# Ghostish/Open3DSOT

Hardware: NVIDIA H100
Metric: template-search pairs/sec, BAT-Car fwd+bwd (higher is better)
Workload: dtype f32

## Files before the change

### open3dsot_b200/csrc/pwmlp_tc.cu

```cuda
#include <type_traits>
#include "common.cuh"
#include "lift.cuh"
#include "tc_ptx.cuh"
#include "../../include/o3d_b200.h"

namespace {

struct TcAct {
    const float* x; int ld; const float* scale; const float* shift; int relu;
    struct Coef { float4 s, t; bool on; };
    template <int R> struct Batch { float4 v[R]; };
    __device__ __forceinline__ Coef prep(int k, int K) const {
        Coef c;
        c.on = k < K;
        c.s = make_float4(1.f, 1.f, 1.f, 1.f);
        c.t = make_float4(0.f, 0.f, 0.f, 0.f);
        if (c.on && scale) { c.s = ld4g(scale + k); c.t = ld4g(shift + k); }
        return c;
    }
    template <int R>
    __device__ __forceinline__ void fetch(Batch<R>& b, int p0, int stride, int P, int k, int K) const {
        const int kk = k < K ? k : 0;
#pragma unroll
        for (int i = 0; i < R; ++i) {
// ... 210 lines not shown
                s2 = fmaf(v[j], v[j], s2);
            }
            if (S > 0) {
                float gm = v[0], gn = v[0];
                int ga = 0, gb = 0;
#pragma unroll
                for (int j = 1; j < 16; ++j) {
                    if (v[j] > gm) { gm = v[j]; ga = j; }
                    if (v[j] < gn) { gn = v[j]; gb = j; }
                }
                const int s0 = pbase & smask;
                if (s0 == 0) { mx = gm; ax = ga; mn = gn; an = gb; }
                else {
                    if (gm > mx) { mx = gm; ax = s0 + ga; }
                    if (gn < mn) { mn = gn; an = s0 + gb; }
                }
                if (s0 + 16 == S) {
                    const size_t o = (size_t)(pbase >> log2S) * ldp + ch;
                    ymax[o] = mx; ymin[o] = mn; arg[o] = ax | (an << 16);
                }
            }
        } else {
#pragma unroll
            for (int j = 0; j < 16; ++j) {
                if (pbase + j >= P) break;
                const float v = __uint_as_float(r[j]) + bv;
                if (yp) yp[(size_t)j * ldy] = v;
                s1 += v;
                s2 = fmaf(v, v, s2);
                if (S > 0) {
                    const int s = (pbase + j) & smask;
                    if (s == 0) { mx = -INFINITY; mn = INFINITY; ax = an = 0; }
                    if (v > mx) { mx = v; ax = s; }
                    if (v < mn) { mn = v; an = s; }
                    if (s == smask) {
                        const size_t o = (size_t)((pbase + j) >> log2S) * ldp + ch;
                        ymax[o] = mx; ymin[o] = mn; arg[o] = ax | (an << 16);
                    }
                }
            }
        }
        d1 += (double)s1;
        d2 += (double)s2;
    }
    __device__ __forceinline__ void end(int ch, int Nw) {
        if (sum && ch < Nw) {
            atomicAdd(sum + ch, d1);
            atomicAdd(sumsq + ch, d2);
        }
    }
};

template <int LD, bool LIFT = false>
struct TcDgradEpi {
    float* out; int ldo; const float* yprev; int ldyp; const float* scale; const float* shift; int relu;
    double* s1g; double* s2y;
    LiftView lv;
    float sc, sh; double d1, d2;
    float yv[16];
    float u0, u1, u2, u3; const int32_t* gs; const float4* ss;
    __device__ __forceinline__ bool lifted() const { return LIFT; }
    __device__ __forceinline__ void begin(int ch, int Nw) {
        d1 = d2 = 0.0;
        sc = (scale && ch < Nw) ? scale[ch] : 1.f;
        sh = (shift && ch < Nw) ? shift[ch] : 0.f;
        if constexpr (LIFT) {
            const bool on = lv.u && ch < Nw;
            u0 = on ? lv.u[ch] : 0.f; u1 = on ? lv.u[lv.ldz + ch] : 0.f; u2 = on ? lv.u[2 * lv.ldz + ch] : 0.f; u3 = on ? lv.u[3 * lv.ldz + ch] : 0.f;
            gs = nullptr;
        }
    }
    __device__ __forceinline__ const int32_t* lift_gidx() const { return LIFT ? lv.gidx : nullptr; }
    __device__ __forceinline__ const float* lift_s() const { return LIFT ? lv.s : nullptr; }
    __device__ __forceinline__ void set_tile(const int32_t* g, const float4* s4) { if constexpr (LIFT) { gs = g; ss = s4; } }
    __device__ __forceinline__ void prefetch_lift(int ch, int pbase, int col, int P) {
#pragma unroll
        for (int j = 0; j < 16; ++j) {
            const float z = lv.z ? __ldg(lv.z + (size_t)gs[col + j] * lv.ldz + ch) : 0.f;
            const float4 sv = lv.s ? ss[col + j] : make_float4(0.f, 0.f, 0.f, 0.f);
            yv[j] = lift_val(z, sv, u0, u1, u2, u3);
        }
    }
    __device__ __forceinline__ void prefetch(int ch, int Nw, int pbase, int P) {
        if (ch >= Nw) return;
        if constexpr (LIFT) { prefetch_lift(ch, pbase, pbase & (TC_N - 1), P); return; }
        if (!yprev) return;
        if (pbase + 16 <= P) {
            const float* yp = yprev + (size_t)pbase * ldyp + ch;
            const size_t st = LD ? (size_t)LD : (size_t)ldyp;
#pragma unroll
            for (int j = 0; j < 16; ++j) yv[j] = __ldg(yp + j * st);
        } else {
#pragma unroll
            for (int j = 0; j < 16; ++j) {
                const int pj = min(pbase + j, P - 1);
                yv[j] = __ldg(yprev + (size_t)pj * ldyp + ch);
            }
        }
    }
    __device__ __forceinline__ void group(const uint32_t (&r)[16], int ch, int Nw, int pbase, int P) {
        if (ch >= Nw) return;
        float s1 = 0.f, s2 = 0.f;
        float* op = out + (size_t)pbase * ldo + ch;
        if (pbase + 16 <= P) {
            float v[16];
#pragma unroll
            for (int j = 0; j < 16; ++j) v[j] = __uint_as_float(r[j]);
            if (yprev || lifted()) {
                if (relu) {
#pragma unroll
                    for (int j = 0; j < 16; ++j) v[j] = fmaf(yv[j], sc, sh) > 0.f ? v[j] : 0.f;
                }
#pragma unroll
                for (int j = 0; j < 16; ++j) s2 = fmaf(v[j], yv[j], s2);
            }
            const size_t st = LD ? (size_t)LD : (size_t)ldo;
#pragma unroll
            for (int j = 0; j < 16; ++j) {
                s1 += v[j];
                op[j * st] = v[j];
            }
        } else {
#pragma unroll
            for (int j = 0; j < 16; ++j) {
                if (pbase + j >= P) break;
                float v = __uint_as_float(r[j]);
                if (yprev || lifted()) {
                    if (relu && !(fmaf(yv[j], sc, sh) > 0.f)) v = 0.f;
                    s2 = fmaf(v, yv[j], s2);
                }
                s1 += v;
                op[(size_t)j * ldo] = v;
            }
        }
        d1 += (double)s1;
        d2 += (double)s2;
    }
    __device__ __forceinline__ void end(int ch, int Nw) {
        if (s1g && ch < Nw) {
            atomicAdd(s1g + ch, d1);
            atomicAdd(s2y + ch, d2);
        }
    }
};

constexpr int TC_STAGES = 2;
constexpr int TC_STAGE_BYTES = 4 * TILE_BYTES;
constexpr int TC_EPI_LD = 68;
constexpr int TC_EPI_BYTES = TC_M * TC_EPI_LD * 4;
constexpr int TC_THREADS = 512;
constexpr int TC_SMEM = TC_STAGES * TC_STAGE_BYTES + 2 * TC_EPI_BYTES + 1024 + 256 + 1024 + 4096;

template <int R>
__device__ __forceinline__ void stage_acc(const float (&acc)[R], float* stg, int ld) {
    const int w = (threadIdx.x >> 5) & 3, lane = threadIdx.x & 31;
#pragma unroll
    for (int i = 0; i < R; ++i) {
        const int row = 16 * w + (lane >> 2) + 8 * ((i >> 1) & 1), col = 8 * (i >> 2) + 2 * (lane & 3) + (i & 1);
        stg[col * ld + row] = acc[i];
    }
}

template <class BLoad, class Epi>
__global__ void __launch_bounds__(TC_THREADS, 1)
    pw_tc_kernel(BLoad bl, const uint8_t* __restrict__ wtiles, int P, int K, int Nw, int nkb, Epi epi, int rev) {
    constexpr bool BF = is_bf16<BLoad>::value;
    constexpr int WBYTES = BF ? BF_TILE_BYTES : 2 * TILE_BYTES;
    extern __shared__ uint8_t smem_raw[];
    uint8_t* smem = reinterpret_cast<uint8_t*>((reinterpret_cast<uintptr_t>(smem_raw) + 1023) & ~(uintptr_t)1023);
    uint8_t* tail = smem + TC_STAGES * TC_STAGE_BYTES + 2 * TC_EPI_BYTES;
    uint64_t* full = reinterpret_cast<uint64_t*>(tail);
    uint64_t* empty = full + TC_STAGES;

    const int warp = threadIdx.x >> 5, lane = threadIdx.x & 31;
    const int mt0 = blockIdx.y;
    const int n_ptiles = (P + TC_N - 1) / TC_N;
    auto tile_of = [&](int t) { return rev ? n_ptiles - 1 - t : t; };

    if (threadIdx.x == 0) {
        for (int s = 0; s < TC_STAGES; ++s) {
            o3d_mbar_init(full + s, 256 + 1);
            o3d_mbar_init(empty + s, 8);
        }
        o3d_fence_mbar_init();
    }
    __syncthreads();

    if (warp < 8) {
        const int h = warp >> 2;
        const int tw = threadIdx.x & 127;
        const int ch = mt0 * TC_M + tw;
        float* stg = reinterpret_cast<float*>(smem + TC_STAGES * TC_STAGE_BYTES + h * TC_EPI_BYTES);
        int32_t* gsm = reinterpret_cast<int32_t*>(tail + 256);
        float4* ssm = reinterpret_cast<float4*>(tail + 256 + 1024);
        epi.begin(ch, Nw);
        int stage = 0, phase = 0, buf = 0;
        for (int t = blockIdx.x; t < n_ptiles; t += gridDim.x) {
            const int pt0 = tile_of(t) * TC_N;
            {
                const int32_t* gi = epi.lift_gidx();
                const float* si = epi.lift_s();
                if (gi || si) {
                    const int pp = min(pt0 + tw, P - 1);
                    if (gi && h == 0) gsm[buf * TC_N + tw] = __ldg(gi + pp);
                    if (si && h == 1) ssm[buf * TC_N + tw] = ld4g(si + (size_t)pp * 4);
                    asm volatile("bar.sync 1, 256;" ::: "memory");
                    epi.set_tile(gsm + buf * TC_N, ssm + buf * TC_N);
                }
            }
            const int pb = pt0 + h * 64;
            epi.prefetch(ch, Nw, pb, P);
            float acc[64];
#pragma unroll
            for (int i = 0; i < 64; ++i) acc[i] = 0.f;
            for (int kb = 0; kb < nkb; ++kb) {
                o3d_mbar_wait(full + stage, phase);
                const uint32_t sb = o3d_smem_u32(smem + stage * TC_STAGE_BYTES);
                wgmma_fence_acc(acc);
                wgmma_fence();
                if constexpr (BF) {
                    const uint32_t xb = sb + 2 * TILE_BYTES + h * (BF_TILE_BYTES / 2);
                    wgmma_bf16_kblock<128>(acc, make_desc_sw64(xb), make_desc_sw64(sb), kb == 0);
                } else {
                    const uint32_t xb = sb + 2 * TILE_BYTES + h * (TILE_BYTES / 2);
                    wgmma_3xtf32_kblock<128>(acc, make_desc(xb), make_desc(xb + TILE_BYTES), make_desc(sb), make_desc(sb + TILE_BYTES),
                                             kb == 0);
                }
                wgmma_commit();
                wgmma_wait<0>();
                wgmma_fence_acc(acc);
                if (lane == 0) o3d_mbar_arrive(empty + stage);
                if (++stage == TC_STAGES) { stage = 0; phase ^= 1; }
            }
            asm volatile("bar.sync %0, 128;" ::"r"(2 + h) : "memory");
            stage_acc(acc, stg, TC_EPI_LD);
            asm volatile("bar.sync %0, 128;" ::"r"(2 + h) : "memory");
            const float* row = stg + tw * TC_EPI_LD;
#pragma unroll 1
            for (int cg = 0; cg < 4; ++cg) {
                uint32_t r[16];
#pragma unroll
                for (int j = 0; j < 4; ++j) {
                    const float4 v = *reinterpret_cast<const float4*>(row + cg * 16 + 4 * j);
                    r[4 * j] = __float_as_uint(v.x); r[4 * j + 1] = __float_as_uint(v.y);
                    r[4 * j + 2] = __float_as_uint(v.z); r[4 * j + 3] = __float_as_uint(v.w);
                }
                epi.group(r, ch, Nw, pb + cg * 16, P);
                if (cg + 1 < 4) epi.prefetch(ch, Nw, pb + (cg + 1) * 16, P);
            }
            buf ^= 1;
        }
        epi.end(ch, Nw);
    } else {
        const int pt = (warp - 8) * 32 + lane;
        const int chunk = pt & 7;
        const int row0 = (pt >> 3) * 4;
        int stage = 0, phase = 0;
        struct Cur { int t, kb, p0; };
        auto advance = [&](Cur& c) {
            if (++c.kb == nkb) {
                c.kb = 0;
                c.t += gridDim.x;
                if (c.t < n_ptiles) c.p0 = tile_of(c.t) * TC_N;
            }
        };
        using Batch4 = typename BLoad::template Batch<4>;
        auto issue = [&](Batch4& r, typename BLoad::Coef& cf, const Cur& c) {
            if (c.t >= n_ptiles) return;
            const int k = c.kb * TC_K + chunk * 4;
            cf = bl.prep(k, K);
            bl.fetch(r, c.p0 + row0, 1, P, k, K);
        };
        Cur c0{(int)blockIdx.x, 0, 0};
        if (c0.t < n_ptiles) c0.p0 = tile_of(c0.t) * TC_N;
        Batch4 r0{};
        typename BLoad::Coef f0 = bl.prep(chunk * 4, K);
        issue(r0, f0, c0);
        if (pt == 0 && c0.t < n_ptiles) bl.prefetch_rows(c0.p0, TC_N, P);
        while (c0.t < n_ptiles) {
            o3d_mbar_wait(empty + stage, phase ^ 1);
            if (pt == 0) {
                o3d_mbar_expect_tx(full + stage, WBYTES);
                o3d_bulk_g2s(smem + stage * TC_STAGE_BYTES, wtiles + ((size_t)mt0 * nkb + c0.kb) * WBYTES, WBYTES, full + stage);
                const int tn = c0.t + (int)gridDim.x;
                if (c0.kb == 0 && tn < n_ptiles) bl.prefetch_rows(tile_of(tn) * TC_N, TC_N, P);
            }
            uint8_t* xhi = smem + stage * TC_STAGE_BYTES + 2 * TILE_BYTES;
            uint8_t* xlo = xhi + TILE_BYTES;
#pragma unroll
            for (int i = 0; i < 4; ++i) {
                const float4 v = bl.finish(r0, f0, i, c0.p0 + row0 + i, P);
                if constexpr (BF) {
                    *reinterpret_cast<uint2*>(xhi + sw64(row0 + i, chunk >> 1) + (chunk & 1) * 8) = pack_bf16x4(v);
                } else {
                    const uint32_t off = sw128(row0 + i, chunk);
                    *reinterpret_cast<float4*>(xhi + off) = hi_part(v);
                    *reinterpret_cast<float4*>(xlo + off) = lo_part(v);
                }
            }
            o3d_fence_proxy_async();
            o3d_mbar_arrive(full + stage);
            if (++stage == TC_STAGES) { stage = 0; phase ^= 1; }
            advance(c0);
            issue(r0, f0, c0);
        }
    }
}

constexpr int WG_STAGES = 3;
constexpr int WG_AHEAD = 4;
constexpr int WG_THREADS = 512;
constexpr int WG_SMEM = WG_STAGES * 4 * TILE_BYTES + 1024 + 256;

template <class L>
__device__ __forceinline__ void store_transposed(const L& ld, const typename L::template Batch<4>& raw, const typename L::Coef& cf,
                                                 uint8_t* hi, int c_local, int p_first, int prow0, int pend) {
#pragma unroll
    for (int i = 0; i < 4; ++i) {
        const int pl = prow0 + 8 * i;
        const float4 v = ld.finish(raw, cf, i, p_first + pl, pend);
        const float e[4] = {v.x, v.y, v.z, v.w};
#pragma unroll
        for (int j = 0; j < 4; ++j) {
            const uint32_t off = sw128(c_local + j, pl >> 2) + (uint32_t)((pl & 3) * 4);
            const float h = hi1(e[j]);
            *reinterpret_cast<float*>(hi + off) = h;
            *reinterpret_cast<float*>(hi + TILE_BYTES + off) = e[j] - h;
        }
    }
}

constexpr int WG_BF_SUB = TC_K * TC_BF_ROW;
constexpr int WG_BF_X = 4 * WG_BF_SUB;

template <class L>
__device__ __forceinline__ void store_rows_bf16(const L& ld, const typename L::template Batch<4>& raw, const typename L::Coef& cf,
                                                uint8_t* img, int sub, int c_local, int p_first, int prow0, int pend) {
#pragma unroll
    for (int i = 0; i < 4; ++i) {
        const int pl = prow0 + 8 * i;
        st_bf16_row4(img, sub, pl, c_local, ld.finish(raw, cf, i, p_first + pl, pend));
    }
}

template <class XB>
__global__ void __launch_bounds__(WG_THREADS, 1)
    pw_wgrad_tc_kernel(TcDy da, XB xb, int P, int M, int N, int chunk, float* __restrict__ part) {
    constexpr bool BF = is_bf16<XB>::value;
    extern __shared__ uint8_t smem_raw[];
    uint8_t* smem = reinterpret_cast<uint8_t*>((reinterpret_cast<uintptr_t>(smem_raw) + 1023) & ~(uintptr_t)1023);
    uint64_t* full = reinterpret_cast<uint64_t*>(smem + WG_STAGES * 4 * TILE_BYTES);
    uint64_t* empty = full + WG_STAGES;

    const int warp = threadIdx.x >> 5, lane = threadIdx.x & 31;
    const int m0 = blockIdx.z * TC_M, n0 = blockIdx.y * TC_N;
    const int pbeg = blockIdx.x * chunk, pend = min(P, pbeg + chunk);
    const int nkb = pend > pbeg ? (pend - pbeg + TC_K - 1) / TC_K : 0;
    auto kpos = [&](int i) { return pbeg + i * TC_K; };

    if (threadIdx.x == 0) {
        for (int s = 0; s < WG_STAGES; ++s) {
            o3d_mbar_init(full + s, 256);
            o3d_mbar_init(empty + s, 8);
        }
        o3d_fence_mbar_init();
    }
    __syncthreads();

    if (warp < 8) {
        const int h = warp >> 2, w = warp & 3;
        float acc[64];
#pragma unroll
        for (int i = 0; i < 64; ++i) acc[i] = 0.f;
        int stage = 0, phase = 0;
        for (int kb = 0; kb < nkb; ++kb) {
            o3d_mbar_wait(full + stage, phase);
            const uint32_t sb = o3d_smem_u32(smem + stage * 4 * TILE_BYTES);
            wgmma_fence_acc(acc);
            wgmma_fence();
            if constexpr (BF) {
                const uint32_t ab = sb + h * 2 * WG_BF_SUB;
#pragma unroll
                for (int ks = 0; ks < 2; ++ks)
                    wgmma_bf16_tt_n128(acc, make_desc_sw64_mn(ab + ks * 1024, WG_BF_SUB),
                                       make_desc_sw64_mn(sb + WG_BF_X + ks * 1024, WG_BF_SUB), (kb == 0 && ks == 0) ? 0u : 1u);
            } else {
                const uint32_t ab = sb + h * (TILE_BYTES / 2);
                wgmma_3xtf32_kblock<128>(acc, make_desc(ab), make_desc(ab + TILE_BYTES), make_desc(sb + 2 * TILE_BYTES),
                                         make_desc(sb + 3 * TILE_BYTES), kb == 0);
            }
            wgmma_commit();
            wgmma_wait<0>();
            wgmma_fence_acc(acc);
            if (lane == 0) o3d_mbar_arrive(empty + stage);
            if (++stage == WG_STAGES) { stage = 0; phase ^= 1; }
        }
        const int Mt = TC_M * (int)gridDim.z, Nt = TC_N * (int)gridDim.y;
        float* __restrict__ out = part + (size_t)blockIdx.x * Mt * Nt;
#pragma unroll
        for (int i = 0; i < 64; i += 4) {
#pragma unroll
            for (int rr = 0; rr < 2; ++rr) {
                const int m = m0 + h * 64 + 16 * w + (lane >> 2) + 8 * rr, n = n0 + 8 * (i >> 2) + 2 * (lane & 3);
                *reinterpret_cast<float2*>(out + (size_t)m * Nt + n) = make_float2(acc[i + 2 * rr], acc[i + 2 * rr + 1]);
            }
        }
    } else {
        const int pw = warp - 8;
        const int c4 = pw * 4 + (lane & 3), prow0 = lane >> 2;
        const bool pt0 = pw == 0 && lane == 0;
        TcDy::Batch<4> ra = {};
        typename XB::template Batch<4> rb = {};
        auto fetch = [&](int kb) {
            da.fetch(ra, kpos(kb) + prow0, 8, pend, m0 + c4 * 4, M);
            xb.fetch(rb, kpos(kb) + prow0, 8, pend, n0 + c4 * 4, N);
        };
        auto prefetch = [&](int kb) {
            if (pt0 && kb < nkb) {
                da.prefetch_rows(kpos(kb), TC_K, pend);
                xb.prefetch_rows(kpos(kb), TC_K, pend);
            }
        };
        int stage = 0, phase = 0;
        for (int kb = 0; kb < WG_AHEAD; ++kb) prefetch(kb);
        if (nkb > 0) fetch(0);
        for (int kb = 0; kb < nkb; ++kb) {
            prefetch(kb + WG_AHEAD);
            o3d_mbar_wait(empty + stage, phase ^ 1);
            uint8_t* sbase = smem + stage * 4 * TILE_BYTES;
            if constexpr (BF) {
                store_rows_bf16(da, ra, da.prep(m0 + c4 * 4, M), sbase, WG_BF_SUB, c4 * 4, kpos(kb), prow0, pend);
                store_rows_bf16(xb, rb, xb.prep(n0 + c4 * 4, N), sbase + WG_BF_X, WG_BF_SUB, c4 * 4, kpos(kb), prow0, pend);
            } else {
                store_transposed(da, ra, da.prep(m0 + c4 * 4, M), sbase, c4 * 4, kpos(kb), prow0, pend);
                store_transposed(xb, rb, xb.prep(n0 + c4 * 4, N), sbase + 2 * TILE_BYTES, c4 * 4, kpos(kb), prow0, pend);
            }
            o3d_fence_proxy_async();
            o3d_mbar_arrive(full + stage);
            if (kb + 1 < nkb) fetch(kb + 1);
            if (++stage == WG_STAGES) { stage = 0; phase ^= 1; }
        }
    }
}

__global__ void __launch_bounds__(256)
    wgrad_reduce_kernel(const float* __restrict__ part, int splits, int Mt, int Nt, int M, int N, float* __restrict__ dW,
                        int lddw) {
    const int sub = threadIdx.x & 7;
    const int n4 = (blockIdx.x * 32 + (threadIdx.x >> 3)) * 4, m = blockIdx.y;
    float4 acc = make_float4(0.f, 0.f, 0.f, 0.f);
    if (n4 < N && m < M) {
        const float* p = part + (size_t)m * Nt + n4;
        for (int s = sub; s < splits; s += 8) {
            const float4 v = __ldg(reinterpret_cast<const float4*>(p + (size_t)s * Mt * Nt));
            acc.x += v.x; acc.y += v.y; acc.z += v.z; acc.w += v.w;
        }
    }
#pragma unroll
    for (int o = 4; o >= 1; o >>= 1) {
        acc.x += __shfl_xor_sync(0xFFFFFFFFu, acc.x, o); acc.y += __shfl_xor_sync(0xFFFFFFFFu, acc.y, o);
        acc.z += __shfl_xor_sync(0xFFFFFFFFu, acc.z, o); acc.w += __shfl_xor_sync(0xFFFFFFFFu, acc.w, o);
    }
    if (sub == 0 && n4 < N && m < M) {
        float* o = dW + (size_t)m * lddw + n4;
        o[0] += acc.x;
        if (n4 + 1 < N) o[1] += acc.y;
        if (n4 + 2 < N) o[2] += acc.z;
        if (n4 + 3 < N) o[3] += acc.w;
    }
}

constexpr int BW_TP = 64;
constexpr int BW_THREADS = 384;
constexpr int BW_DY = 0, BW_XT = 64 * 1024, BW_W = 128 * 1024, BW_TAIL = 192 * 1024;
constexpr int BW_SMEM = BW_TAIL + 256 + 1024 + 4096 + 1024;
constexpr int BW_BF_SUB = BW_TP * TC_BF_ROW;

template <class XB, int N>
__global__ void __launch_bounds__(BW_THREADS, 1)
    pw_bwd_tc_kernel(TcDy da, XB xb, const uint8_t* __restrict__ wtiles, int P, int M, TcDgradEpi<N, is_lift<XB>::value> epi,
                     float* __restrict__ part) {
    constexpr bool BF = is_bf16<XB>::value;
    constexpr int NH = N / 2;
    constexpr int WSTAGE = BF ? NH * TC_BF_ROW : 2 * NH * 128;
    extern __shared__ uint8_t smem_raw[];
    uint8_t* smem = reinterpret_cast<uint8_t*>((reinterpret_cast<uintptr_t>(smem_raw) + 1023) & ~(uintptr_t)1023);
    uint8_t* tail = smem + BW_TAIL;
    uint64_t* dy_full = reinterpret_cast<uint64_t*>(tail);
    uint64_t* dy_empty = dy_full + 1;
    uint64_t* xt_full = dy_full + 2;
    uint64_t* xt_empty = dy_full + 3;
    uint64_t* wfull = dy_full + 4;

    const int warp = threadIdx.x >> 5, lane = threadIdx.x & 31;
    const int nkb = M / TC_K;
    const int n_ptiles = (P + BW_TP - 1) / BW_TP;
    const int my_tiles = blockIdx.x < n_ptiles ? (n_ptiles - 1 - blockIdx.x) / gridDim.x + 1 : 0;

    if (threadIdx.x == 0) {
        o3d_mbar_init(dy_full, 128);
        o3d_mbar_init(dy_empty, 8);
        o3d_mbar_init(xt_full, 128);
        o3d_mbar_init(xt_empty, 8);
        for (int s = 0; s < 4; ++s) o3d_mbar_init(wfull + s, 1);
        o3d_fence_mbar_init();
    }
    __syncthreads();

    if (warp < 8) {
        const int h = warp >> 2, w = warp & 3, tw = threadIdx.x & 127;
        uint8_t* wring = smem + BW_W + h * 2 * WSTAGE;
        const int n_witems = my_tiles * nkb;
        auto load_w = [&](int item) {
            const int s = item & 1;
            o3d_mbar_expect_tx(wfull + 2 * h + s, WSTAGE);
            if constexpr (BF) {
                const uint8_t* src = wtiles + (size_t)(item % nkb) * BF_TILE_BYTES + h * NH * TC_BF_ROW;
                o3d_bulk_g2s(wring + s * WSTAGE, src, WSTAGE, wfull + 2 * h + s);
            } else {
                const uint8_t* src = wtiles + (size_t)(item % nkb) * (2 * TILE_BYTES) + h * NH * 128;
                o3d_bulk_g2s(wring + s * WSTAGE, src, NH * 128, wfull + 2 * h + s);
                o3d_bulk_g2s(wring + s * WSTAGE + NH * 128, src + TILE_BYTES, NH * 128, wfull + 2 * h + s);
            }
        };
        if (tw == 0) {
            if (n_witems > 0) load_w(0);
            if (n_witems > 1) load_w(1);
        }
        const bool do_w = 64 * h < M;
        const int n_local = h * NH + (tw % NH);
        const int q = tw / NH;
        constexpr int PPT = NH / 2;
        float* stg = reinterpret_cast<float*>(smem + BW_XT + h * (NH * TC_EPI_LD * 4));
        int32_t* gsm = reinterpret_cast<int32_t*>(tail + 256);
        float4* ssm = reinterpret_cast<float4*>(tail + 256 + 1024);
        epi.begin(n_local, N);
        float wacc[N / 2];
#pragma unroll
        for (int i = 0; i < N / 2; ++i) wacc[i] = 0.f;
        int witem = 0, tphase = 0, buf = 0;
        for (int t = blockIdx.x; t < n_ptiles; t += gridDim.x) {
            const int pt0 = t * BW_TP;
            {
                const int32_t* gi = epi.lift_gidx();
                const float* si = epi.lift_s();
                if (gi || si) {
                    if (tw < BW_TP) {
                        const int pp = min(pt0 + tw, P - 1);
                        const int slot = buf * TC_N + ((pt0 + tw) & (TC_N - 1));
                        if (gi && h == 0) gsm[slot] = __ldg(gi + pp);
                        if (si && h == 1) ssm[slot] = ld4g(si + (size_t)pp * 4);
                    }
                    asm volatile("bar.sync 1, 256;" ::: "memory");
                    epi.set_tile(gsm + buf * TC_N, ssm + buf * TC_N);
                }
            }
            const int pb = pt0 + q * PPT;
            float dacc[NH / 2];
#pragma unroll
            for (int i = 0; i < NH / 2; ++i) dacc[i] = 0.f;
            o3d_mbar_wait(dy_full, tphase);
            for (int kb = 0; kb < nkb; ++kb, ++witem) {
                o3d_mbar_wait(wfull + 2 * h + (witem & 1), (witem >> 1) & 1);
                const uint32_t bb = o3d_smem_u32(wring + (witem & 1) * WSTAGE);
                wgmma_fence_acc(dacc);
                wgmma_fence();
                if constexpr (BF) {
                    wgmma_bf16_kblock<NH>(dacc, make_desc_sw64(o3d_smem_u32(smem + BW_DY + kb * BW_BF_SUB)), make_desc_sw64(bb), kb == 0);
                } else {
                    const uint32_t ab = o3d_smem_u32(smem + BW_DY + kb * TILE_BYTES);
                    wgmma_3xtf32_kblock<NH>(dacc, make_desc(ab), make_desc(ab + TILE_BYTES / 2), make_desc(bb), make_desc(bb + NH * 128),
                                            kb == 0);
                }
                wgmma_commit();
                wgmma_wait<0>();
                wgmma_fence_acc(dacc);
                asm volatile("bar.sync %0, 128;" ::"r"(2 + h) : "memory");
                if (tw == 0 && witem + 2 < n_witems) load_w(witem + 2);
            }
            o3d_mbar_wait(xt_full, tphase);
            if constexpr (BF) {
                if (do_w) {
                    const uint32_t ab = o3d_smem_u32(smem + BW_DY + 2 * h * BW_BF_SUB), xb0 = o3d_smem_u32(smem + BW_XT);
                    wgmma_fence_acc(wacc);
                    wgmma_fence();
#pragma unroll
                    for (int ks = 0; ks < BW_TP / 16; ++ks) {
                        const uint64_t ad = make_desc_sw64_mn(ab + ks * 1024, BW_BF_SUB), bd = make_desc_sw64_mn(xb0 + ks * 1024, BW_BF_SUB);
                        if constexpr (N == 128) wgmma_bf16_tt_n128(wacc, ad, bd, 1u);
                        else wgmma_bf16_tt_n64(wacc, ad, bd, 1u);
                    }
                    wgmma_commit();
                    wgmma_wait<0>();
                    wgmma_fence_acc(wacc);
                }
            } else if (do_w) {
                const int mr = 16 * w + (lane >> 2);
                const uint8_t* dyk = smem + BW_DY + (2 * h + (w >> 1)) * (TILE_BYTES);
                const int mc = mr & 31;
                const uint32_t xt = o3d_smem_u32(smem + BW_XT);
#pragma unroll 1
                for (int ks = 0; ks < BW_TP / 8; ++ks) {
                    uint32_t ahi[4], alo[4];
#pragma unroll
                    for (int i = 0; i < 4; ++i) {
                        const int p = ks * 8 + (lane & 3) + 4 * (i >> 1), m = mc + 8 * (i & 1);
                        const uint32_t off = sw128(p, m >> 2) + 4 * (m & 3);
                        ahi[i] = *reinterpret_cast<const uint32_t*>(dyk + off);
                        alo[i] = *reinterpret_cast<const uint32_t*>(dyk + TILE_BYTES / 2 + off);
                    }
                    const uint32_t xb0 = xt + (ks >> 2) * (2 * TILE_BYTES) + (ks & 3) * 32;
                    const uint64_t bhi = make_desc(xb0), blo = make_desc(xb0 + TILE_BYTES);
                    wgmma_fence_acc(wacc);
                    wgmma_fence();
                    if constexpr (N == 128) {
                        wgmma_tf32_rs_n128(wacc, alo, bhi);
                        wgmma_tf32_rs_n128(wacc, ahi, blo);
                        wgmma_tf32_rs_n128(wacc, ahi, bhi);
                    } else {
                        wgmma_tf32_rs_n64(wacc, alo, bhi);
                        wgmma_tf32_rs_n64(wacc, ahi, blo);
                        wgmma_tf32_rs_n64(wacc, ahi, bhi);
                    }
                    wgmma_commit();
                    wgmma_wait<0>();
                    wgmma_fence_acc(wacc);
                }
            }
            __syncwarp();
            if (lane == 0) o3d_mbar_arrive(dy_empty);
            epi.prefetch(n_local, N, pb, P);
            asm volatile("bar.sync 4, 256;" ::: "memory");
            stage_acc(dacc, stg, TC_EPI_LD);
            asm volatile("bar.sync %0, 128;" ::"r"(2 + h) : "memory");
            const float* row = stg + (tw % NH) * TC_EPI_LD + q * PPT;
#pragma unroll 1
            for (int cg = 0; cg < PPT / 16; ++cg) {
                uint32_t r[16];
#pragma unroll
                for (int j = 0; j < 4; ++j) {
                    const float4 v = *reinterpret_cast<const float4*>(row + cg * 16 + 4 * j);
                    r[4 * j] = __float_as_uint(v.x); r[4 * j + 1] = __float_as_uint(v.y);
                    r[4 * j + 2] = __float_as_uint(v.z); r[4 * j + 3] = __float_as_uint(v.w);
                }
                epi.group(r, n_local, N, pb + cg * 16, P);
                if (cg + 1 < PPT / 16) epi.prefetch(n_local, N, pb + (cg + 1) * 16, P);
            }
            __syncwarp();
            if (lane == 0) o3d_mbar_arrive(xt_empty);
            tphase ^= 1;
            buf ^= 1;
        }
        epi.end(n_local, N);
        if (do_w) {
            float* __restrict__ out = part + (size_t)blockIdx.x * TC_M * TC_N;
#pragma unroll
            for (int i = 0; i < N / 2; i += 4) {
#pragma unroll
                for (int rr = 0; rr < 2; ++rr) {
                    const int m = 64 * h + 16 * w + (lane >> 2) + 8 * rr, n = 8 * (i >> 2) + 2 * (lane & 3);
                    *reinterpret_cast<float2*>(out + (size_t)m * TC_N + n) = make_float2(wacc[i + 2 * rr], wacc[i + 2 * rr + 1]);
                }
            }
        }
    } else {
        const int pt = threadIdx.x - 256;
        const int chunk = pt & 7, row0 = (pt >> 3) * 4;
        const int pw = warp - 8, c4 = pw * 4 + (lane & 3), prow0 = lane >> 2;
        constexpr int NXH = N / 64;
        const int n_items_x = 2 * NXH;
        struct It { int t, i; };
        TcDy::Batch<4> ra{};
        typename XB::template Batch<4> rb{};
        It ca{(int)blockIdx.x, 0}, cb{(int)blockIdx.x, 0};
        auto fetch_a = [&](const It& c) {
            if (c.t < n_ptiles) da.fetch(ra, c.t * BW_TP + row0, 1, P, c.i * TC_K + chunk * 4, M);
        };
        auto fetch_b = [&](const It& c) {
            if (c.t < n_ptiles)
                xb.fetch(rb, c.t * BW_TP + (c.i >> (NXH - 1)) * TC_K + prow0, 8, P, (c.i & (NXH - 1)) * 64 + c4 * 4, N);
        };
        fetch_a(ca);
        fetch_b(cb);
        if (pt == 0 && ca.t < n_ptiles) { da.prefetch_rows(ca.t * BW_TP, BW_TP, P); xb.prefetch_rows(ca.t * BW_TP, BW_TP, P); }
        int tphase = 0;
        for (int t = blockIdx.x; t < n_ptiles; t += gridDim.x) {
            const int pt0 = t * BW_TP;
            if (pt == 0) {
                const int tn = t + (int)gridDim.x;
                if (tn < n_ptiles) { da.prefetch_rows(tn * BW_TP, BW_TP, P); xb.prefetch_rows(tn * BW_TP, BW_TP, P); }
            }
            o3d_mbar_wait(dy_empty, tphase ^ 1);
            for (int kb = 0; kb < nkb; ++kb) {
                const int k = kb * TC_K + chunk * 4;
                const TcDy::Coef cf = da.prep(k, M);
                if constexpr (BF) {
#pragma unroll
                    for (int i = 0; i < 4; ++i)
                        st_bf16_row4(smem + BW_DY + kb * BW_BF_SUB, 0, row0 + i, chunk * 4, da.finish(ra, cf, i, pt0 + row0 + i, P));
                } else {
                    uint8_t* hi = smem + BW_DY + kb * TILE_BYTES;
#pragma unroll
                    for (int i = 0; i < 4; ++i) {
                        const float4 v = da.finish(ra, cf, i, pt0 + row0 + i, P);
                        const uint32_t off = sw128(row0 + i, chunk);
                        *reinterpret_cast<float4*>(hi + off) = hi_part(v);
                        *reinterpret_cast<float4*>(hi + TILE_BYTES / 2 + off) = lo_part(v);
                    }
                }
                if (++ca.i == nkb) { ca.i = 0; ca.t += gridDim.x; }
                fetch_a(ca);
            }
            o3d_fence_proxy_async();
            o3d_mbar_arrive(dy_full);
            o3d_mbar_wait(xt_empty, tphase ^ 1);
            for (int it = 0; it < n_items_x; ++it) {
                const int j = it >> (NXH - 1), cl = (it & (NXH - 1)) * 64 + c4 * 4;
                if constexpr (BF)
                    store_rows_bf16(xb, rb, xb.prep(cl, N), smem + BW_XT + j * (TC_K * TC_BF_ROW), BW_BF_SUB, cl, pt0 + j * TC_K, prow0, P);
                else
                    store_transposed(xb, rb, xb.prep(cl, N), smem + BW_XT + j * (2 * TILE_BYTES), cl, pt0 + j * TC_K, prow0, P);
                if (++cb.i == n_items_x) { cb.i = 0; cb.t += gridDim.x; }
                fetch_b(cb);
            }
            o3d_fence_proxy_async();
            o3d_mbar_arrive(xt_full);
            tphase ^= 1;
        }
    }
}

__global__ void w_pretile_kernel(const float* __restrict__ W, int ld, int rows, int K, int nkb, uint8_t* __restrict__ out) {
    const int m_tile = blockIdx.y, kb = blockIdx.x;
    uint8_t* dst = out + ((size_t)m_tile * nkb + kb) * (2 * TILE_BYTES);
    for (int id = threadIdx.x; id < TC_M * 8; id += blockDim.x) {
        const int r = id >> 3, c = id & 7;
        const int row = m_tile * TC_M + r, k = kb * TC_K + c * 4;
        float4 v = make_float4(0.f, 0.f, 0.f, 0.f);
        if (row < rows && k < K) v = *reinterpret_cast<const float4*>(W + (size_t)row * ld + k);
        const uint32_t off = sw128(r, c);
        *reinterpret_cast<float4*>(dst + off) = hi_part(v);
        *reinterpret_cast<float4*>(dst + TILE_BYTES + off) = lo_part(v);
    }
}

inline int ilog2_exact(int v) { int l = 0; while ((1 << l) < v) ++l; return l; }

template <class BLoad, class Epi>
int launch_tc(BLoad bl, const uint8_t* wtiles, int P, int K, int Nw, Epi epi, bool reverse, cudaStream_t st, const char* name) {
    auto kern = pw_tc_kernel<BLoad, Epi>;
    O3D_CUDA(cudaFuncSetAttribute(kern, cudaFuncAttributeMaxDynamicSharedMemorySize, TC_SMEM), name);
    const int gy = (Nw + TC_M - 1) / TC_M;
    const int nkb = (K + TC_K - 1) / TC_K;
    const int n_ptiles = (P + TC_N - 1) / TC_N;
    int gx = o3d_num_sms() / gy;
    if (gx < 1) gx = 1;
    if (gx > n_ptiles) gx = n_ptiles;
    kern<<<dim3(gx, gy), TC_THREADS, TC_SMEM, st>>>(bl, wtiles, P, K, Nw, nkb, epi, reverse);
    O3D_CHECK_LAUNCH(name);
    return O3D_OK;
}

template <int LD, class BLoad>
int launch_fwd(const BLoad& bl, const void* wtiles, const float* bias, int P, int K, int Nw, float* y, int ldy, double* sum,
               double* sumsq, int S, float* ymax, float* ymin, int32_t* arg, int ldp, bool reverse, cudaStream_t st) {
    TcFwdEpi<LD> ep{};
    ep.y = y; ep.ldy = ldy; ep.bias = bias; ep.sum = sum; ep.sumsq = sumsq;
    ep.S = S; ep.ymax = ymax; ep.ymin = ymin; ep.arg = arg; ep.ldp = ldp;
    ep.log2S = 0;
    while ((1 << ep.log2S) < S) ++ep.log2S;
    return launch_tc(bl, (const uint8_t*)wtiles, P, K, Nw, ep, reverse, st, "o3d_pw_fwd_tc");
}

template <int LD, bool LIFT = false, class BL>
int launch_dgrad(const BL& bl, const void* wtiles_t, int P, int Cout, int Cin, float* out, int ldo, const float* yprev,
                 int ldyp, const float* pscale, const float* pshift, int prelu, double* s1, double* s2y, cudaStream_t st,
                 const LiftView* lv = nullptr) {
    if constexpr (!LIFT) {
        if (lv) return launch_dgrad<LD, true>(bl, wtiles_t, P, Cout, Cin, out, ldo, yprev, ldyp, pscale, pshift, prelu, s1, s2y, st, lv);
    }
    TcDgradEpi<LD, LIFT> ep{};
    if (lv) ep.lv = *lv;
    ep.out = out; ep.ldo = ldo; ep.yprev = yprev; ep.ldyp = ldyp; ep.scale = pscale; ep.shift = pshift; ep.relu = prelu;
    ep.s1g = s1; ep.s2y = s2y;
    return launch_tc(bl, (const uint8_t*)wtiles_t, P, Cout, Cin, ep, false, st, "o3d_pw_dgrad_tc");
}

}

extern "C" long long o3d_pw_tc_wtile_bytes(int rows, int K) {
    const long long mt = (rows + TC_M - 1) / TC_M, nkb = (K + TC_K - 1) / TC_K;
    return mt * nkb * 2 * TILE_BYTES;
}

extern "C" int o3d_pw_tc_pretile(const float* w, int ldw, int rows, int K, void* wtiles, void* stream) {
    O3D_REQUIRE(w && wtiles, O3D_ERR_ARG, "o3d_pw_tc_pretile: null pointer");
    O3D_REQUIRE((K & 3) == 0 && (ldw & 3) == 0, O3D_ERR_ARG, "o3d_pw_tc_pretile: K and ldw must be multiples of 4");
    O3D_REQUIRE(((uintptr_t)wtiles & 15) == 0 && ((uintptr_t)w & 15) == 0, O3D_ERR_ALIGN, "o3d_pw_tc_pretile: alignment");
    const int mt = (rows + TC_M - 1) / TC_M, nkb = (K + TC_K - 1) / TC_K;
    w_pretile_kernel<<<dim3(nkb, mt), 256, 0, (cudaStream_t)stream>>>(w, ldw, rows, K, nkb, (uint8_t*)wtiles);
    O3D_CHECK_LAUNCH("o3d_pw_tc_pretile");
    return O3D_OK;
}

int o3d_pw_fwd_tc_dir(const float* x, int ldx, const float* in_scale, const float* in_shift, int in_relu, const void* wtiles,
                      const float* bias, int P, int K, int N, float* y, int ldy, double* sum, double* sumsq, int S, float* ymax,
                      float* ymin, int32_t* arg, int ldp, void* stream, bool reverse, bool bf16) {
    O3D_REQUIRE(x && wtiles, O3D_ERR_ARG, "o3d_pw_fwd_tc: null pointer");
    O3D_REQUIRE(P >= 0 && K >= 4 && N >= 1 && (K & 3) == 0 && (ldx & 3) == 0, O3D_ERR_ARG, "o3d_pw_fwd_tc: bad sizes");
    O3D_REQUIRE(S == 0 || (P % S == 0 && 64 % S == 0 && ymax && ymin && arg), O3D_ERR_ARG,
                "o3d_pw_fwd_tc: pooling group size must divide 64 and P");
    if (P == 0) return O3D_OK;
    const int Nw = (N + 3) & ~3;
    TcAct bl{x, ldx, in_scale, in_shift, in_relu};
    cudaStream_t st = (cudaStream_t)stream;
    if (bf16) {
        Bf16<TcAct> bb{bl};
#define O3D_FWD_ARGS bb, wtiles, bias, P, K, Nw, y, ldy, sum, sumsq, S, ymax, ymin, arg, ldp, reverse, st
        if (ldy == 64) return launch_fwd<64>(O3D_FWD_ARGS);
        if (ldy == 128) return launch_fwd<128>(O3D_FWD_ARGS);
        if (ldy == 256) return launch_fwd<256>(O3D_FWD_ARGS);
        return launch_fwd<0>(O3D_FWD_ARGS);
#undef O3D_FWD_ARGS
    }
#define O3D_FWD_ARGS bl, wtiles, bias, P, K, Nw, y, ldy, sum, sumsq, S, ymax, ymin, arg, ldp, reverse, st
    if (ldy == 64) return launch_fwd<64>(O3D_FWD_ARGS);
    if (ldy == 128) return launch_fwd<128>(O3D_FWD_ARGS);
    if (ldy == 256) return launch_fwd<256>(O3D_FWD_ARGS);
    return launch_fwd<0>(O3D_FWD_ARGS);
#undef O3D_FWD_ARGS
}

extern "C" int o3d_pw_fwd_tc(const float* x, int ldx, const float* in_scale, const float* in_shift, int in_relu,
                             const void* wtiles, const float* bias, int P, int K, int N, float* y, int ldy, double* sum,
                             double* sumsq, int S, float* ymax, float* ymin, int32_t* arg, int ldp, void* stream) {
    return o3d_pw_fwd_tc_dir(x, ldx, in_scale, in_shift, in_relu, wtiles, bias, P, K, N, y, ldy, sum, sumsq, S, ymax, ymin, arg,
                             ldp, stream, false, false);
}

namespace {
int dgrad_tc_impl(const float* g, int ldg, const float* y, int ldy, const float* a, const float* b, const float* cc,
                  const float* dpool, const int32_t* sel, int S, int ldp, const void* wtiles_t, int P, int Cout, int Cin,
                  float* out, int ldo, const float* yprev, int ldyp, const float* pscale, const float* pshift, int prelu,
                  double* s1, double* s2y, void* stream, const LiftView* lv, bool bf16) {
    O3D_REQUIRE((g || dpool) && wtiles_t && out, O3D_ERR_ARG, "o3d_pw_dgrad_tc: null pointer");
    O3D_REQUIRE((Cout & 3) == 0 && (Cin & 3) == 0, O3D_ERR_ARG, "o3d_pw_dgrad_tc: channel counts must be multiples of 4");
    if (P == 0) return O3D_OK;
    TcDy bl{g, ldg, y, ldy, a, b, cc, dpool, sel, S > 0 ? S : 1, ldp, ilog2_exact(S > 0 ? S : 1)};
    cudaStream_t st = (cudaStream_t)stream;
    const int ld = (!yprev || ldyp == ldo) ? ldo : 0;
    auto run = [&](const auto& ldr) {
#define O3D_DG_ARGS ldr, wtiles_t, P, Cout, Cin, out, ldo, yprev, ldyp, pscale, pshift, prelu, s1, s2y, st, lv
        if (ld == 64) return launch_dgrad<64>(O3D_DG_ARGS);
        if (ld == 128) return launch_dgrad<128>(O3D_DG_ARGS);
        if (ld == 256) return launch_dgrad<256>(O3D_DG_ARGS);
        return launch_dgrad<0>(O3D_DG_ARGS);
#undef O3D_DG_ARGS
    };
    return bf16 ? run(Bf16<TcDy>{bl}) : run(bl);
}
}

int o3d_pw_dgrad_tc_prec(const float* g, int ldg, const float* y, int ldy, const float* a, const float* b, const float* cc,
                         const float* dpool, const int32_t* sel, int S, int ldp, const void* wtiles_t, int P, int Cout, int Cin,
                         float* out, int ldo, const float* yprev, int ldyp, const float* pscale, const float* pshift, int prelu,
                         double* s1, double* s2y, void* stream, bool bf16) {
    return dgrad_tc_impl(g, ldg, y, ldy, a, b, cc, dpool, sel, S, ldp, wtiles_t, P, Cout, Cin, out, ldo, yprev, ldyp, pscale,
                         pshift, prelu, s1, s2y, stream, nullptr, bf16);
}

extern "C" int o3d_pw_dgrad_tc(const float* g, int ldg, const float* y, int ldy, const float* a, const float* b,
                               const float* cc, const float* dpool, const int32_t* sel, int S, int ldp,
                               const void* wtiles_t, int P, int Cout, int Cin, float* out, int ldo, const float* yprev,
                               int ldyp, const float* pscale, const float* pshift, int prelu, double* s1, double* s2y,
                               void* stream) {
    return dgrad_tc_impl(g, ldg, y, ldy, a, b, cc, dpool, sel, S, ldp, wtiles_t, P, Cout, Cin, out, ldo, yprev, ldyp, pscale,
// ... 216 lines not shown
```

Before: 3022.

## Deepen weight ring, stage dgrad epilogue separately, double-buffer producer fetches in bwd

The backward TC kernel's weight ring grows from two to up to eight stages. When every k-block fits, the weights stay resident and the per-k-block barrier and reload are skipped. The dgrad epilogue now stages into its own small smem region in rounds, so xt_empty can be released before the epilogue runs instead of after it. The producer warps hold two register batches in flight for the non-lift inputs, giving more memory-level parallelism. This adds register pressure and extra named barriers per round.

```diff
diff --git a/open3dsot_b200/csrc/pwmlp_tc.cu b/open3dsot_b200/csrc/pwmlp_tc.cu
--- a/open3dsot_b200/csrc/pwmlp_tc.cu
+++ b/open3dsot_b200/csrc/pwmlp_tc.cu
@@ -386,11 +386,11 @@
 constexpr int TC_SMEM = TC_STAGES * TC_STAGE_BYTES + 2 * TC_EPI_BYTES + 1024 + 256 + 1024 + 4096;
 
 template <int R>
-__device__ __forceinline__ void stage_acc(const float (&acc)[R], float* stg, int ld) {
-    const int w = (threadIdx.x >> 5) & 3, lane = threadIdx.x & 31;
+__device__ __forceinline__ void stage_acc(const float (&acc)[R], float* stg, int ld, int slot) {
+    const int lane = threadIdx.x & 31;
 #pragma unroll
     for (int i = 0; i < R; ++i) {
-        const int row = 16 * w + (lane >> 2) + 8 * ((i >> 1) & 1), col = 8 * (i >> 2) + 2 * (lane & 3) + (i & 1);
+        const int row = 16 * slot + (lane >> 2) + 8 * ((i >> 1) & 1), col = 8 * (i >> 2) + 2 * (lane & 3) + (i & 1);
         stg[col * ld + row] = acc[i];
     }
 }
@@ -467,7 +467,7 @@
                 if (++stage == TC_STAGES) { stage = 0; phase ^= 1; }
             }
             asm volatile("bar.sync %0, 128;" ::"r"(2 + h) : "memory");
-            stage_acc(acc, stg, TC_EPI_LD);
+            stage_acc(acc, stg, TC_EPI_LD, (threadIdx.x >> 5) & 3);
             asm volatile("bar.sync %0, 128;" ::"r"(2 + h) : "memory");
             const float* row = stg + tw * TC_EPI_LD;
 #pragma unroll 1
@@ -707,7 +707,10 @@
 constexpr int BW_TP = 64;
 constexpr int BW_THREADS = 384;
 constexpr int BW_DY = 0, BW_XT = 64 * 1024, BW_W = 128 * 1024, BW_TAIL = 192 * 1024;
-constexpr int BW_SMEM = BW_TAIL + 256 + 1024 + 4096 + 1024;
+constexpr int BW_WRING = 32 * 1024;
+constexpr int BW_STG = BW_TAIL + 256 + 1024 + 4096;
+constexpr int BW_STG_FLOATS = 64 * (32 + 4);
+constexpr int BW_SMEM = BW_STG + 2 * BW_STG_FLOATS * 4 + 1024;
 constexpr int BW_BF_SUB = BW_TP * TC_BF_ROW;
 
 template <class XB, int N>
@@ -717,6 +720,7 @@
     constexpr bool BF = is_bf16<XB>::value;
     constexpr int NH = N / 2;
     constexpr int WSTAGE = BF ? NH * TC_BF_ROW : 2 * NH * 128;
+    constexpr int WSTAGES = (BW_WRING / WSTAGE) < 8 ? (BW_WRING / WSTAGE) : 8;
     extern __shared__ uint8_t smem_raw[];
     uint8_t* smem = reinterpret_cast<uint8_t*>((reinterpret_cast<uintptr_t>(smem_raw) + 1023) & ~(uintptr_t)1023);
     uint8_t* tail = smem + BW_TAIL;
@@ -736,36 +740,39 @@
         o3d_mbar_init(dy_empty, 8);
         o3d_mbar_init(xt_full, 128);
         o3d_mbar_init(xt_empty, 8);
-        for (int s = 0; s < 4; ++s) o3d_mbar_init(wfull + s, 1);
+        for (int s = 0; s < 2 * WSTAGES; ++s) o3d_mbar_init(wfull + s, 1);
         o3d_fence_mbar_init();
     }
     __syncthreads();
 
     if (warp < 8) {
         const int h = warp >> 2, w = warp & 3, tw = threadIdx.x & 127;
-        uint8_t* wring = smem + BW_W + h * 2 * WSTAGE;
+        uint8_t* wring = smem + BW_W + h * BW_WRING;
+        uint64_t* wbar = wfull + h * WSTAGES;
         const int n_witems = my_tiles * nkb;
+        const bool resident = WSTAGES % nkb == 0;
         auto load_w = [&](int item) {
-            const int s = item & 1;
-            o3d_mbar_expect_tx(wfull + 2 * h + s, WSTAGE);
+            const int s = item % WSTAGES;
+            o3d_mbar_expect_tx(wbar + s, WSTAGE);
             if constexpr (BF) {
                 const uint8_t* src = wtiles + (size_t)(item % nkb) * BF_TILE_BYTES + h * NH * TC_BF_ROW;
-                o3d_bulk_g2s(wring + s * WSTAGE, src, WSTAGE, wfull + 2 * h + s);
+                o3d_bulk_g2s(wring + s * WSTAGE, src, WSTAGE, wbar + s);
             } else {
                 const uint8_t* src = wtiles + (size_t)(item % nkb) * (2 * TILE_BYTES) + h * NH * 128;
-                o3d_bulk_g2s(wring + s * WSTAGE, src, NH * 128, wfull + 2 * h + s);
-                o3d_bulk_g2s(wring + s * WSTAGE + NH * 128, src + TILE_BYTES, NH * 128, wfull + 2 * h + s);
+                o3d_bulk_g2s(wring + s * WSTAGE, src, NH * 128, wbar + s);
+                o3d_bulk_g2s(wring + s * WSTAGE + NH * 128, src + TILE_BYTES, NH * 128, wbar + s);
             }
         };
-        if (tw == 0) {
-            if (n_witems > 0) load_w(0);
-            if (n_witems > 1) load_w(1);
-        }
+        if (tw == 0)
+            for (int i = 0; i < WSTAGES && i < n_witems; ++i) load_w(i);
         const bool do_w = 64 * h < M;
         const int n_local = h * NH + (tw % NH);
         const int q = tw / NH;
         constexpr int PPT = NH / 2;
-        float* stg = reinterpret_cast<float*>(smem + BW_XT + h * (NH * TC_EPI_LD * 4));
+        constexpr int ROUNDS = PPT / 16;
+        constexpr int SLD = BW_TP / ROUNDS + 4;
+        static_assert(NH * SLD <= BW_STG_FLOATS, "epilogue staging");
+        float* stg = reinterpret_cast<float*>(smem + BW_STG) + h * BW_STG_FLOATS;
         int32_t* gsm = reinterpret_cast<int32_t*>(tail + 256);
         float4* ssm = reinterpret_cast<float4*>(tail + 256 + 1024);
         epi.begin(n_local, N);
@@ -795,8 +802,9 @@
             for (int i = 0; i < NH / 2; ++i) dacc[i] = 0.f;
             o3d_mbar_wait(dy_full, tphase);
             for (int kb = 0; kb < nkb; ++kb, ++witem) {
-                o3d_mbar_wait(wfull + 2 * h + (witem & 1), (witem >> 1) & 1);
-                const uint32_t bb = o3d_smem_u32(wring + (witem & 1) * WSTAGE);
+                const int ws = witem % WSTAGES;
+                o3d_mbar_wait(wbar + ws, resident ? 0 : (witem / WSTAGES) & 1);
+                const uint32_t bb = o3d_smem_u32(wring + ws * WSTAGE);
                 wgmma_fence_acc(dacc);
                 wgmma_fence();
                 if constexpr (BF) {
@@ -809,8 +817,10 @@
                 wgmma_commit();
                 wgmma_wait<0>();
                 wgmma_fence_acc(dacc);
-                asm volatile("bar.sync %0, 128;" ::"r"(2 + h) : "memory");
-                if (tw == 0 && witem + 2 < n_witems) load_w(witem + 2);
+                if (!resident) {
+                    asm volatile("bar.sync %0, 128;" ::"r"(2 + h) : "memory");
+                    if (tw == 0 && witem + WSTAGES < n_witems) load_w(witem + WSTAGES);
+                }
             }
             o3d_mbar_wait(xt_full, tphase);
             if constexpr (BF) {
@@ -862,26 +872,30 @@
                 }
             }
             __syncwarp();
-            if (lane == 0) o3d_mbar_arrive(dy_empty);
+            if (lane == 0) {
+                o3d_mbar_arrive(dy_empty);
+                o3d_mbar_arrive(xt_empty);
+            }
             epi.prefetch(n_local, N, pb, P);
-            asm volatile("bar.sync 4, 256;" ::: "memory");
-            stage_acc(dacc, stg, TC_EPI_LD);
-            asm volatile("bar.sync %0, 128;" ::"r"(2 + h) : "memory");
-            const float* row = stg + (tw % NH) * TC_EPI_LD + q * PPT;
-#pragma unroll 1
-            for (int cg = 0; cg < PPT / 16; ++cg) {
-                uint32_t r[16];
+            const float* row = stg + (tw % NH) * SLD + 16 * q;
+            uint32_t r[ROUNDS][16];
+#pragma unroll
+            for (int cg = 0; cg < ROUNDS; ++cg) {
+                asm volatile("bar.sync %0, 128;" ::"r"(2 + h) : "memory");
+                if (w % ROUNDS == cg) stage_acc(dacc, stg, SLD, w / ROUNDS);
+                asm volatile("bar.sync %0, 128;" ::"r"(2 + h) : "memory");
 #pragma unroll
                 for (int j = 0; j < 4; ++j) {
-                    const float4 v = *reinterpret_cast<const float4*>(row + cg * 16 + 4 * j);
-                    r[4 * j] = __float_as_uint(v.x); r[4 * j + 1] = __float_as_uint(v.y);
-                    r[4 * j + 2] = __float_as_uint(v.z); r[4 * j + 3] = __float_as_uint(v.w);
-                }
-                epi.group(r, n_local, N, pb + cg * 16, P);
-                if (cg + 1 < PPT / 16) epi.prefetch(n_local, N, pb + (cg + 1) * 16, P);
-            }
-            __syncwarp();
-            if (lane == 0) o3d_mbar_arrive(xt_empty);
+                    const float4 v = *reinterpret_cast<const float4*>(row + 4 * j);
+                    r[cg][4 * j] = __float_as_uint(v.x); r[cg][4 * j + 1] = __float_as_uint(v.y);
+                    r[cg][4 * j + 2] = __float_as_uint(v.z); r[cg][4 * j + 3] = __float_as_uint(v.w);
+                }
+            }
+#pragma unroll
+            for (int cg = 0; cg < ROUNDS; ++cg) {
+                epi.group(r[cg], n_local, N, pb + cg * 16, P);
+                if (cg + 1 < ROUNDS) epi.prefetch(n_local, N, pb + (cg + 1) * 16, P);
+            }
             tphase ^= 1;
             buf ^= 1;
         }
@@ -903,20 +917,25 @@
         const int pw = warp - 8, c4 = pw * 4 + (lane & 3), prow0 = lane >> 2;
         constexpr int NXH = N / 64;
         const int n_items_x = 2 * NXH;
+        constexpr int AY = is_lift<XB>::value ? 1 : 2, AX = AY;
         struct It { int t, i; };
-        TcDy::Batch<4> ra{};
-        typename XB::template Batch<4> rb{};
+        TcDy::Batch<4> ra[AY] = {};
+        typename XB::template Batch<4> rb[AX] = {};
         It ca{(int)blockIdx.x, 0}, cb{(int)blockIdx.x, 0};
-        auto fetch_a = [&](const It& c) {
-            if (c.t < n_ptiles) da.fetch(ra, c.t * BW_TP + row0, 1, P, c.i * TC_K + chunk * 4, M);
+        auto fetch_a = [&](TcDy::Batch<4>& r, It& c) {
+            if (c.t < n_ptiles) da.fetch(r, c.t * BW_TP + row0, 1, P, c.i * TC_K + chunk * 4, M);
+            if (++c.i == nkb) { c.i = 0; c.t += gridDim.x; }
         };
-        auto fetch_b = [&](const It& c) {
+        auto fetch_b = [&](typename XB::template Batch<4>& r, It& c) {
             if (c.t < n_ptiles)
-                xb.fetch(rb, c.t * BW_TP + (c.i >> (NXH - 1)) * TC_K + prow0, 8, P, (c.i & (NXH - 1)) * 64 + c4 * 4, N);
+                xb.fetch(r, c.t * BW_TP + (c.i >> (NXH - 1)) * TC_K + prow0, 8, P, (c.i & (NXH - 1)) * 64 + c4 * 4, N);
+            if (++c.i == n_items_x) { c.i = 0; c.t += gridDim.x; }
         };
-        fetch_a(ca);
-        fetch_b(cb);
         if (pt == 0 && ca.t < n_ptiles) { da.prefetch_rows(ca.t * BW_TP, BW_TP, P); xb.prefetch_rows(ca.t * BW_TP, BW_TP, P); }
+#pragma unroll
+        for (int u = 0; u < AY; ++u) fetch_a(ra[u], ca);
+#pragma unroll
+        for (int u = 0; u < AX; ++u) fetch_b(rb[u], cb);
         int tphase = 0;
         for (int t = blockIdx.x; t < n_ptiles; t += gridDim.x) {
             const int pt0 = t * BW_TP;
@@ -925,37 +944,44 @@
                 if (tn < n_ptiles) { da.prefetch_rows(tn * BW_TP, BW_TP, P); xb.prefetch_rows(tn * BW_TP, BW_TP, P); }
             }
             o3d_mbar_wait(dy_empty, tphase ^ 1);
-            for (int kb = 0; kb < nkb; ++kb) {
-                const int k = kb * TC_K + chunk * 4;
-                const TcDy::Coef cf = da.prep(k, M);
-                if constexpr (BF) {
-#pragma unroll
-                    for (int i = 0; i < 4; ++i)
-                        st_bf16_row4(smem + BW_DY + kb * BW_BF_SUB, 0, row0 + i, chunk * 4, da.finish(ra, cf, i, pt0 + row0 + i, P));
-                } else {
-                    uint8_t* hi = smem + BW_DY + kb * TILE_BYTES;
-#pragma unroll
-                    for (int i = 0; i < 4; ++i) {
-                        const float4 v = da.finish(ra, cf, i, pt0 + row0 + i, P);
-                        const uint32_t off = sw128(row0 + i, chunk);
-                        *reinterpret_cast<float4*>(hi + off) = hi_part(v);
-                        *reinterpret_cast<float4*>(hi + TILE_BYTES / 2 + off) = lo_part(v);
+            for (int kb0 = 0; kb0 < nkb; kb0 += AY) {
+#pragma unroll
+                for (int u = 0; u < AY; ++u) {
+                    const int kb = kb0 + u;
+                    const int k = kb * TC_K + chunk * 4;
+                    const TcDy::Coef cf = da.prep(k, M);
+                    if constexpr (BF) {
+#pragma unroll
+                        for (int i = 0; i < 4; ++i)
+                            st_bf16_row4(smem + BW_DY + kb * BW_BF_SUB, 0, row0 + i, chunk * 4, da.finish(ra[u], cf, i, pt0 + row0 + i, P));
+                    } else {
+                        uint8_t* hi = smem + BW_DY + kb * TILE_BYTES;
+#pragma unroll
+                        for (int i = 0; i < 4; ++i) {
+                            const float4 v = da.finish(ra[u], cf, i, pt0 + row0 + i, P);
+                            const uint32_t off = sw128(row0 + i, chunk);
+                            *reinterpret_cast<float4*>(hi + off) = hi_part(v);
+                            *reinterpret_cast<float4*>(hi + TILE_BYTES / 2 + off) = lo_part(v);
+                        }
                     }
-                }
-                if (++ca.i == nkb) { ca.i = 0; ca.t += gridDim.x; }
-                fetch_a(ca);
+                    fetch_a(ra[u], ca);
+                }
             }
             o3d_fence_proxy_async();
             o3d_mbar_arrive(dy_full);
             o3d_mbar_wait(xt_empty, tphase ^ 1);
-            for (int it = 0; it < n_items_x; ++it) {
-                const int j = it >> (NXH - 1), cl = (it & (NXH - 1)) * 64 + c4 * 4;
-                if constexpr (BF)
-                    store_rows_bf16(xb, rb, xb.prep(cl, N), smem + BW_XT + j * (TC_K * TC_BF_ROW), BW_BF_SUB, cl, pt0 + j * TC_K, prow0, P);
-                else
-                    store_transposed(xb, rb, xb.prep(cl, N), smem + BW_XT + j * (2 * TILE_BYTES), cl, pt0 + j * TC_K, prow0, P);
-                if (++cb.i == n_items_x) { cb.i = 0; cb.t += gridDim.x; }
-                fetch_b(cb);
+            for (int it0 = 0; it0 < n_items_x; it0 += AX) {
+#pragma unroll
+                for (int u = 0; u < AX; ++u) {
+                    const int it = it0 + u;
+                    const int j = it >> (NXH - 1), cl = (it & (NXH - 1)) * 64 + c4 * 4;
+                    if constexpr (BF)
+                        store_rows_bf16(xb, rb[u], xb.prep(cl, N), smem + BW_XT + j * (TC_K * TC_BF_ROW), BW_BF_SUB, cl, pt0 + j * TC_K, prow0,
+                                        P);
+                    else
+                        store_transposed(xb, rb[u], xb.prep(cl, N), smem + BW_XT + j * (2 * TILE_BYTES), cl, pt0 + j * TC_K, prow0, P);
+                    fetch_b(rb[u], cb);
+                }
             }
             o3d_fence_proxy_async();
             o3d_mbar_arrive(xt_full);
```

Result: faster. 3052 (median of 6 runs) (+1.0%).
